# bridgedp/hunter_bipedal_control

Measured on NVIDIA H100. Metric: MPC+WBC control-step solves/sec (Hunter N=100), higher is better.
Workload: dtype f64

## Files before the change

hunter_bipedal_control_b200/csrc/hb_api.cu:

```cuda
#include <cuda_runtime.h>
#include <math.h>
#include <stdio.h>
#include <stdlib.h>
#include <string.h>

#include <new>

#include "../../include/hunter_b200.h"
#include "hb_common.cuh"
#include "hb_mpc.cuh"
#include "hb_planner.h"
#include <algorithm>
#include <climits>
#include <string>
#include <utility>
#include <atomic>
#include <mutex>
#include <cstring>
#include <thread>
#include <vector>
#include "hb_qp.cuh"
#include "hb_rbd.cuh"
#include "hb_sqp.cuh"
#include "hb_wbc.cuh"
// ... 214 lines not shown
      ctx_->base = (int)lo;
      rc = copy(lo, hi, true);
      if (!rc) rc = body(Chunk{c, lo, hi, (int)(hi - lo)});
      if (!rc) rc = copy(lo, hi, false);
    }
    ctx_->stream = ctx_->stream_main;
    ctx_->base = 0;
    return drain(ctx_, rc);
  }

 private:
  struct Slot { const void* src; void* dst; size_t bytes, count; void* dev; bool used; };
  template <class T> Dev<T> add(const void* src, void* dst, size_t per, size_t count, bool used) {
    Slot& s = s_[n_++];
    s = Slot{src, dst, per * sizeof(T), count, nullptr, used};
    return Dev<T>{&s.dev, per};
  }
  size_t place(void* base) {
    size_t off = 0;
    for (int k = 0; k < n_; ++k) if (s_[k].used) s_[k].dev = carve<char>(base, off, s_[k].bytes * s_[k].count);
    return off;
  }
  int copy(size_t lo, size_t hi, bool to_dev) {
    hb_ctx* ctx = ctx_;
    for (int k = 0; k < n_; ++k) {
      const Slot& s = s_[k];
      const size_t off = lo * s.bytes, n = (hi - lo) * s.bytes;
      if (to_dev && s.src) CK(cudaMemcpyAsync(static_cast<char*>(s.dev) + off, static_cast<const char*>(s.src) + off, n, cudaMemcpyHostToDevice, ctx->stream));
      if (!to_dev && s.dst) CK(cudaMemcpyAsync(static_cast<char*>(s.dst) + off, static_cast<char*>(s.dev) + off, n, cudaMemcpyDeviceToHost, ctx->stream));
    }
    return HB_OK;
  }
  hb_ctx* ctx_;
  size_t B_;
  Slot s_[16];
  int n_ = 0;
};

int cycle_chunks(const hb_ctx* ctx, int B, bool overlap) {
  const int c = ctx->cfg.e2e_chunks;
  return c > 0 ? (B >= 64 * c ? c : 1) : ((overlap && B >= 4096) ? 2 : 1);
}

}

extern "C" {

int hb_default_config(hb_config* cfg) {
  if (!cfg) return HB_EINVAL;
  cfg->horizon_N = 100;
  cfg->dt = 0.01;
  cfg->max_batch = 1024;
  cfg->wbc_rho = 1e-8;
  cfg->qp_max_iter = 40;
  cfg->line_search_max_trials = 14;
  cfg->time_horizon = 0.0;
  cfg->event_nodes = 0;
  cfg->e2e_chunks = 0;
  return HB_OK;
}

const char* hb_strerror(int code) {
  switch (code) {
    case HB_OK: return "ok";
    case HB_EINVAL: return "invalid argument";
    case HB_ECUDA: return "CUDA error";
    case HB_ENOMEM: return "out of memory";
    case HB_ECAP: return "batch exceeds context capacity";
    case HB_EPLAN: return "reference planner: swing phase without take-off / touch-down time, or reference capacity exceeded";
    case HB_ECOMM: return "NCCL not available or a collective failed (hb_shard_last_error)";
    default: return "unknown error";
  }
}

int hb_create(const hb_config* cfg, int device, hb_ctx** out) {
  if (!cfg || !out || cfg->horizon_N < 1 || cfg->horizon_N > HB_MAX_HORIZON || cfg->max_batch < 1 || !(cfg->dt > 0.0) || cfg->time_horizon < 0.0) return HB_EINVAL;
  hb_ctx* ctx = new (std::nothrow) hb_ctx();
  if (!ctx) return HB_ENOMEM;
  memset(ctx, 0, sizeof(*ctx));
  ctx->cfg = *cfg;
  ctx->device = device;
  hb_default_wbc_settings(&ctx->wbc);
  if (cudaSetDevice(device) != cudaSuccess) { hb_destroy(ctx); return HB_ECUDA; }
  if (cudaStreamCreateWithFlags(&ctx->stream, cudaStreamNonBlocking) != cudaSuccess) { ctx->stream = nullptr; hb_destroy(ctx); return HB_ECUDA; }
  ctx->stream_main = ctx->stream;
  if (cudaStreamCreateWithFlags(&ctx->stream_aux, cudaStreamNonBlocking) != cudaSuccess) { ctx->stream_aux = nullptr; hb_destroy(ctx); return HB_ECUDA; }
  Model* m = new Model();
  memset(m, 0, sizeof(Model));
  for (int b = 0; b < NBODY; ++b) {
    for (int i = 0; i < 3; ++i) { m->joint_xyz[3 * b + i] = HB_JOINT_XYZ[3 * b + i]; m->com[3 * b + i] = HB_BODY_COM[3 * b + i]; }
    for (int i = 0; i < 9; ++i) m->inertia[9 * b + i] = HB_BODY_INERTIA[9 * b + i];
    m->mass[b] = HB_BODY_MASS[b];
    int code = 0;
    for (int i = 0; i < 3; ++i) if (HB_JOINT_AXIS[3 * b + i] != 0.0) code = (HB_JOINT_AXIS[3 * b + i] > 0 ? 1 : -1) * (i + 1);
    m->joint_axis[b] = code;
  }
  m->total_mass = HB_TOTAL_MASS;
  for (int i = 0; i < 12; ++i) m->contact_offset[i] = HB_CONTACT_OFFSET[i];
  for (int j = 0; j < NJ; ++j) { m->joint_lower[j] = HB_JOINT_LOWER[j]; m->joint_upper[j] = HB_JOINT_UPPER[j]; m->joint_vel_limit[j] = HB_JOINT_VEL_LIMIT[j]; m->torque_limit[j] = HB_WBC_TORQUE_LIMITS[j % 5]; }
  for (int i = 0; i < NX; ++i) m->Q[i] = HB_Q_DIAG[i];
  cudaError_t e = cudaMemcpyToSymbol(c_model, m, sizeof(Model));
  if (e == cudaSuccess) {
    double* dR = nullptr;
    e = dalloc(&dR, NU * NU);
    if (e == cudaSuccess) {
      init_input_cost_kernel<<<1, 32, 0, ctx->stream>>>(dR);
      e = cudaStreamSynchronize(ctx->stream);
      if (e == cudaSuccess) e = cudaMemcpy(m->R, dR, sizeof(double) * NU * NU, cudaMemcpyDeviceToHost);
      if (e == cudaSuccess) e = cudaMemcpyToSymbol(c_model, m, sizeof(Model));
      cudaFree(dR);
    }
  }
  if (e == cudaSuccess) {
    double tab[32 * LQ_LANE_TAB] = {};
    for (int l = 0; l < 32; ++l) {
      double* t = tab + l * LQ_LANE_TAB;
      if (l < NX) t[0] = m->Q[l];
      if (l < 12) t[1] = m->R[l * NU + l];
      if (l >= 12 && l < NU) for (int j = 0; j < NJ; ++j) t[2 + j] = m->R[l * NU + 12 + j];
      if (l < 10) { t[12] = m->joint_lower[l]; t[13] = m->joint_upper[l]; }
      else if (l < 20) { t[12] = -m->joint_vel_limit[l - 10]; t[13] = m->joint_vel_limit[l - 10]; }
    }
    e = cudaMemcpyToSymbol(g_lq_lane, tab, sizeof(tab));
  }
  delete m;
  if (e != cudaSuccess) { ctx->last_cuda = (int)e; hb_destroy(ctx); return HB_ECUDA; }
  const size_t B = cfg->max_batch, N = cfg->horizon_N;
  const int rc = reserve_group(&ctx->scratch_mem, [&](void* m) {
    size_t off = 0;
    ctx->dxt = carve<double>(m, off, B * (N + 1) * NX); ctx->dut = carve<double>(m, off, B * N * NU);
    ctx->perf = carve<double>(m, off, B * 4); ctx->flags = carve<int32_t>(m, off, B);
    ctx->xdes = carve<double>(m, off, B * NX); ctx->udes = carve<double>(m, off, B * NU);
    ctx->wstatus = carve<int32_t>(m, off, B); ctx->witers = carve<int32_t>(m, off, B); ctx->wmode = carve<int32_t>(m, off, B);
    ctx->cyc_xref = carve<double>(m, off, B * (N + 1) * NX); ctx->cyc_swing = carve<double>(m, off, B * (N + 1) * 24);
    ctx->cyc_mode = carve<int32_t>(m, off, B * (N + 1)); ctx->cyc_tk = carve<double>(m, off, B * (N + 1)); ctx->cyc_nn = carve<int32_t>(m, off, B);
    ctx->res = carve_solution(m, off, B, N);
    ctx->res_sol = carve<double>(m, off, B * NWBC); ctx->res_stance = carve<double>(m, off, B * 12);
    return off;
  });
  if (rc) { hb_destroy(ctx); return rc; }
  {
    cudaError_t fe = cudaSuccess;
    auto attr = [&](const void* fn, size_t bytes) { if (fe == cudaSuccess) fe = cudaFuncSetAttribute(fn, cudaFuncAttributeMaxDynamicSharedMemorySize, (int)bytes); };
    attr((const void*)probe_flow_map_kernel, sizeof(ProbeShared));
    attr((const void*)qp_batch_kernel, 200 * 1024);
    attr((const void*)wbc_fused_kernel, wbc_fused_doubles() * sizeof(double));
    attr((const void*)hoqp_kernel, hoqp_smem_bytes());
    attr((const void*)hwbc_fused_kernel, hwbc_fused_bytes());
    attr((const void*)lin_kernel, 4 * sizeof(LinHalf) + sizeof(ChainModel));
    attr((const void*)lq_kernel, sizeof(LqShared));
    attr((const void*)riccati_kernel, sizeof(RicShared));
    attr((const void*)forward_linesearch2_kernel, sizeof(Fw2Shared));
    attr((const void*)warm_shift_kernel, sizeof(double) * ((HB_MAX_HORIZON + 1) * NX + HB_MAX_HORIZON * NU));
    for (const void* fn : {(const void*)wbc_fused_kernel, (const void*)riccati_kernel, (const void*)lq_kernel, (const void*)hwbc_fused_kernel})
      if (fe == cudaSuccess) fe = cudaFuncSetAttribute(fn, cudaFuncAttributePreferredSharedMemoryCarveout, (int)cudaSharedmemCarveoutMaxShared);
    if (fe != cudaSuccess) { ctx->last_cuda = (int)fe; hb_destroy(ctx); return HB_ECUDA; }
  }
  *out = ctx;
  return HB_OK;
}

int hb_destroy(hb_ctx* ctx) {
  if (!ctx) return HB_EINVAL;
  cudaSetDevice(ctx->device);
  void* const mem[] = {ctx->scratch_mem, ctx->sqp_mem, ctx->hoqp_mem, ctx->ro_mem, ctx->re_mem, ctx->goal_mem, ctx->pol_mem, ctx->odom_mem, ctx->arena,
                       ctx->pushes.dev, ctx->variations.dev, ctx->terrains.dev, ctx->goals.dev, ctx->plan_targets.dev, ctx->latencies.dev,
                       ctx->odometry.dev};
  for (void* p : mem) if (p) cudaFree(p);
  if (ctx->pinned) cudaFreeHost(ctx->pinned);
  if (ctx->prof_ev) { for (int i = 0; i < 2 * PROF_MAX; ++i) cudaEventDestroy(ctx->prof_ev[i]); delete[] ctx->prof_ev; delete[] ctx->prof_kind; }
  if (ctx->stream_aux) cudaStreamDestroy(ctx->stream_aux);
  if (ctx->stream_main) cudaStreamDestroy(ctx->stream_main);
  else if (ctx->stream) cudaStreamDestroy(ctx->stream);
  delete ctx;
  return HB_OK;
}

int hb_sync(hb_ctx* ctx) {
  if (!ctx) return HB_EINVAL;
  CK(cudaStreamSynchronize(ctx->stream));
  return HB_OK;
}
int hb_profile_enable(hb_ctx* ctx, int on) {
  if (!ctx) return HB_EINVAL;
  if (set_device(ctx)) return HB_ECUDA;
  if (on && !ctx->prof_ev) {
    ctx->prof_ev = new (std::nothrow) cudaEvent_t[2 * PROF_MAX];
    ctx->prof_kind = new (std::nothrow) int[PROF_MAX];
    if (!ctx->prof_ev || !ctx->prof_kind) return HB_ENOMEM;
    for (int i = 0; i < 2 * PROF_MAX; ++i) CK(cudaEventCreate(&ctx->prof_ev[i]));
  }
  ctx->prof_on = on ? 1 : 0;
  ctx->prof_n = 0;
  return HB_OK;
}

int hb_profile_read(hb_ctx* ctx, double* ms_per_kind, int64_t* count_per_kind) {
  if (!ctx || !ms_per_kind || !count_per_kind) return HB_EINVAL;
  if (set_device(ctx)) return HB_ECUDA;
  CK(cudaStreamSynchronize(ctx->stream));
  for (int k = 0; k < K_NKINDS; ++k) { ms_per_kind[k] = 0.0; count_per_kind[k] = 0; }
  for (int i = 0; i < ctx->prof_n; ++i) {
    float ms = 0.f;
    CK(cudaEventElapsedTime(&ms, ctx->prof_ev[2 * i], ctx->prof_ev[2 * i + 1]));
    ms_per_kind[ctx->prof_kind[i]] += ms;
    count_per_kind[ctx->prof_kind[i]]++;
  }
  ctx->prof_n = 0;
  return HB_OK;
}

const char* hb_last_cuda_error(const hb_ctx* ctx) { return ctx ? cudaGetErrorString((cudaError_t)ctx->last_cuda) : "no context"; }

int64_t hb_launch_count(const hb_ctx* ctx) { return ctx ? ctx->launches : 0; }
int64_t hb_last_reference_upload_bytes(const hb_ctx* ctx) { return ctx ? (int64_t)ctx->last_h2d_bytes : 0; }
void* hb_stream(hb_ctx* ctx) { return ctx ? (void*)ctx->stream : nullptr; }

static int launch_qp(hb_ctx* ctx, int B, int n, int m, const double* H, const double* g, const double* A, const double* lbA, const double* ubA,
                     size_t sH, size_t sA, size_t sB, const int32_t* m_per, double* x, int32_t* status, int32_t* iters) {
  if (!qp_shape_ok(n, m)) return HB_EINVAL;
  const size_t per_warp = qp_workspace_doubles(n) * sizeof(double);
  int wpb = (int)((200 * 1024) / per_warp);
  if (wpb < 1) return HB_EINVAL;
  if (wpb > 1) wpb = 1;
  const int blocks = (B + wpb - 1) / wpb;
  return launch(ctx, K_QP, qp_batch_kernel, blocks, 32 * wpb, per_warp * wpb, B, n, m, H, g, A, lbA, ubA, sH, sA, sB, m_per, ctx->cfg.wbc_rho,
                ctx->cfg.qp_max_iter, x, status, iters);
}

int hb_wbc_qp_batch_dev(hb_ctx* ctx, int B, int n, int m, const double* H, const double* g, const double* A, const double* lbA,
                        const double* ubA, double* x, int32_t* status, int32_t* iters) {
  ENTER(ctx, B, H && g && A && lbA && ubA && x, UNCAPPED);
  return launch_qp(ctx, B, n, m, H, g, A, lbA, ubA, (size_t)n * n, (size_t)m * n, (size_t)m, nullptr, x, status, iters);
}

int hb_wbc_solve_batch_dev(hb_ctx* ctx, int B, const double* x_des, const double* u_des, const double* rbd, const int32_t* mode,
                           const uint8_t* stance_mode, double* sol, int32_t* status) {
  ENTER(ctx, B, x_des && u_des && rbd && mode && sol, CAPPED);
  return launch(ctx, K_QP, wbc_fused_kernel, B, 32, wbc_fused_doubles() * sizeof(double), B, ctx->wbc, x_des, u_des, rbd, mode, stance_mode,
                ctx->cfg.wbc_rho, ctx->cfg.qp_max_iter, sol, status ? status : ctx->wstatus + ctx->base, ctx->witers + ctx->base);
}

int hb_wbc_assemble_batch_dev(hb_ctx* ctx, int B, const double* x_des, const double* u_des, const double* rbd, const int32_t* mode,
                              const uint8_t* stance_mode, double* H, double* g, double* A, double* lbA, double* ubA, int32_t* m_rows) {
  ENTER(ctx, B, x_des && u_des && rbd && mode && H && g && A && lbA && ubA && m_rows, UNCAPPED);
  const int wpb = 4;
  return launch(ctx, K_WBC_ASSEMBLE, wbc_assemble_kernel, (B + wpb - 1) / wpb, 32 * wpb, sizeof(WbcShared) * wpb, B, ctx->wbc, x_des, u_des, rbd, mode,
                stance_mode, H, g, A, lbA, ubA, m_rows);
}

int hb_wbc_qp_rows_batch_dev(hb_ctx* ctx, int B, int n, int m_alloc, const int32_t* m_rows, const double* H, const double* g, const double* A,
                             const double* lbA, const double* ubA, double* x, int32_t* status, int32_t* iters) {
  ENTER(ctx, B, m_rows && H && g && A && lbA && ubA && x, UNCAPPED);
  return launch_qp(ctx, B, n, m_alloc, H, g, A, lbA, ubA, (size_t)n * n, (size_t)m_alloc * n, (size_t)m_alloc, m_rows, x, status, iters);
}

static int hoqp_reserve(hb_ctx* ctx) {
  const size_t Bc = ctx->cfg.max_batch;
  return reserve_group(&ctx->hoqp_mem, [&](void* m) {
    size_t off = 0;
    ctx->hoqp_scratch = carve<double>(m, off, Bc * HQ_SCRATCH);
    return off;
  });
}

int hb_hoqp_solve_batch_dev(hb_ctx* ctx, int B, const hb_hoqp_problem* problems, double* x, double* slack, int32_t* status) {
  ENTER(ctx, B, problems && x, CAPPED);
  const int rc = hoqp_reserve(ctx);
  if (rc) return rc;
  return launch(ctx, K_QP, hoqp_kernel, B, 32, hoqp_smem_bytes(), B, problems, ctx->hoqp_scratch, 2 * ctx->cfg.qp_max_iter, x, slack, status);
}

static int hwbc_tasks_dev(hb_ctx* ctx, int B, const double* x_des, const double* u_des, const double* rbd, const int32_t* mode, hb_hoqp_problem* problems) {
  return launch(ctx, K_WBC_ASSEMBLE, hwbc_tasks_kernel, B, 32, 0, B, ctx->wbc, x_des, u_des, rbd, mode, problems);
}

int hb_hierarchical_wbc_solve_batch_dev(hb_ctx* ctx, int B, const double* x_des, const double* u_des, const double* rbd, const int32_t* mode, double* sol,
                                        int32_t* status) {
  ENTER(ctx, B, x_des && u_des && rbd && mode && sol, CAPPED);
  return launch(ctx, K_QP, hwbc_fused_kernel, B, 32, hwbc_fused_bytes(), B, ctx->wbc, x_des, u_des, rbd, mode, 2 * ctx->cfg.qp_max_iter, sol, status);
}

static int controller_wbc_dev(hb_ctx* ctx, int B, const double* x_des, const double* u_des, const double* rbd, const int32_t* mode,
                              const uint8_t* stance_mode, double* sol, int32_t* status) {
  if (ctx->wbc_form == HB_WBC_HIERARCHICAL)
    return hb_hierarchical_wbc_solve_batch_dev(ctx, B, x_des, u_des, rbd, mode, sol, status ? status : ctx->wstatus + ctx->base);
  return hb_wbc_solve_batch_dev(ctx, B, x_des, u_des, rbd, mode, stance_mode, sol, status);
}

int hb_mpc_cold_start_batch_dev(hb_ctx* ctx, int B, const double* x0, const int32_t* mode, double* x_traj, double* u_traj) {
  ENTER(ctx, B, x0 && mode && x_traj && u_traj, UNCAPPED);
  return launch(ctx, K_UNPROFILED, cold_start_kernel, B, 128, 0, B, ctx->cfg.horizon_N, x0, mode, x_traj, u_traj);
}

static int mpc_solve_impl(hb_ctx* ctx, int B, const double* x0, const double* x_ref, const double* swing_ref, const int32_t* mode,
                          double* x_traj, double* u_traj, hb_solve_info* info, const double* tk, const int32_t* nn) {
  ENTER(ctx, B, x0 && x_ref && swing_ref && mode && x_traj && u_traj && (tk == nullptr) == (nn == nullptr), CAPPED);
  const size_t Bc = ctx->cfg.max_batch, Nc = ctx->cfg.horizon_N;
  int rc = reserve_group(&ctx->sqp_mem, [&](void* m) {
    size_t off = 0;
    ctx->lin = carve<double>(m, off, Bc * Nc * LIN_STRIDE); ctx->proj = carve<double>(m, off, Bc * Nc * PJ_STRIDE);
    ctx->rk = carve<double>(m, off, Bc * Nc * RK_STRIDE);
    return off;
  });
  if (rc) return rc;
  SqpArgs a;
  a.tk = tk; a.nn = nn;
// ... 1209 lines not shown
```

hunter_bipedal_control_b200/csrc/hb_mpc.cuh:

```cuda
#pragma once
#include "hb_common.cuh"
#include "hb_rbd.cuh"

namespace hb {

constexpr int TS = NX * NX;
constexpr int NDIR = 13;

struct Pen { double v, d1, d2; };
__device__ __forceinline__ Pen relaxed_barrier(double h, double mu, double delta) {
  Pen p;
  if (h > delta) { p.v = -mu * log(h); p.d1 = -mu / h; p.d2 = mu / (h * h); }
  else {
    const double z = (h - 2.0 * delta) / delta;
    p.v = mu * (-log(delta) + 0.5 * z * z - 0.5);
    p.d1 = mu * (h - 2.0 * delta) / (delta * delta);
    p.d2 = mu / (delta * delta);
  }
  return p;
}
__device__ __forceinline__ Pen double_sided(double h, double lo, double hi, double mu, double delta) {
  const Pen a = relaxed_barrier(h - lo, mu, delta), b = relaxed_barrier(hi - h, mu, delta);
  Pen p; p.v = a.v + b.v; p.d1 = a.d1 - b.d1; p.d2 = a.d2 + b.d2;
  return p;
}

__device__ inline void flow_map_lane(const double* x, const double* u, double* f, double* epos, double* evel) {
  const Model& md = c_model;
  const double m = md.total_mass;
  double R0[9], ax0[9];
  {
    double sz, cz, sy, cy, sx, cx;
    sincos_t(x[9], sz, cz); sincos_t(x[10], sy, cy); sincos_t(x[11], sx, cx);
    R0[0] = cz * cy; R0[1] = cz * sy * sx - sz * cx; R0[2] = cz * sy * cx + sz * sx;
    R0[3] = sz * cy; R0[4] = sz * sy * sx + cz * cx; R0[5] = sz * sy * cx - cz * sx;
    R0[6] = -sy;     R0[7] = cy * sx;                R0[8] = cy * cx;
    ax0[0] = 0.0; ax0[1] = 0.0; ax0[2] = 1.0;
    ax0[3] = -sz; ax0[4] = cz; ax0[5] = 0.0;
    ax0[6] = cz * cy; ax0[7] = sz * cy; ax0[8] = -sy;
  }
  const double p0[3] = {x[6], x[7], x[8]};
  double P[3] = {0, 0, 0}, Lo[3] = {0, 0, 0}, mc[3] = {0, 0, 0};
  double IO[6] = {0, 0, 0, 0, 0, 0};
  double cp[12], cvj[12];
  auto add_inertia = [&](int b, const double* R, const double* cw) {
    const double mb = md.mass[b];
    const double* I = &md.inertia[9 * b];
    double T[9];
#pragma unroll
    for (int i = 0; i < 3; ++i)
#pragma unroll
      for (int k = 0; k < 3; ++k) T[3 * i + k] = R[3 * i] * I[k] + R[3 * i + 1] * I[3 + k] + R[3 * i + 2] * I[6 + k];
    const double c2 = cw[0] * cw[0] + cw[1] * cw[1] + cw[2] * cw[2];
    IO[0] += T[0] * R[0] + T[1] * R[1] + T[2] * R[2] + mb * (c2 - cw[0] * cw[0]);
    IO[1] += T[0] * R[3] + T[1] * R[4] + T[2] * R[5] - mb * cw[0] * cw[1];
    IO[2] += T[0] * R[6] + T[1] * R[7] + T[2] * R[8] - mb * cw[0] * cw[2];
    IO[3] += T[3] * R[3] + T[4] * R[4] + T[5] * R[5] + mb * (c2 - cw[1] * cw[1]);
    IO[4] += T[3] * R[6] + T[4] * R[7] + T[5] * R[8] - mb * cw[1] * cw[2];
    IO[5] += T[6] * R[6] + T[7] * R[7] + T[8] * R[8] + mb * (c2 - cw[2] * cw[2]);
#pragma unroll
    for (int i = 0; i < 3; ++i) mc[i] += cw[i] * mb;
  };
  {
    double r[3], cw[3];
    rot_const(R0, &md.com[0], r);
#pragma unroll
    for (int i = 0; i < 3; ++i) cw[i] = p0[i] + r[i];
    add_inertia(0, R0, cw);
  }
  for (int leg = 0; leg < 2; ++leg) {
    double R[9], p[3], w[3] = {0, 0, 0}, vl[3] = {0, 0, 0};
#pragma unroll
    for (int i = 0; i < 9; ++i) R[i] = R0[i];
#pragma unroll
    for (int i = 0; i < 3; ++i) p[i] = p0[i];
    for (int j = 0; j < 5; ++j) {
      const int b = 1 + 5 * leg + j;
      double d[3], wxd[3], a[3], sj, cj;
      rot_const(R, &md.joint_xyz[3 * b], d);
      cross(w, d, wxd);
#pragma unroll
      for (int i = 0; i < 3; ++i) { p[i] += d[i]; vl[i] += wxd[i]; }
      sincos_t(x[11 + b], sj, cj);
      joint_rotate_sc(R, md.joint_axis[b], sj, cj, a);
      const double vb = u[11 + b];
#pragma unroll
      for (int i = 0; i < 3; ++i) w[i] += a[i] * vb;
      double r[3], wxr[3], vc[3], cw[3], l[3], wl[3], Iwl[3], Iw[3];
      rot_const(R, &md.com[3 * b], r);
      cross(w, r, wxr);
      const double mb = md.mass[b];
#pragma unroll
      for (int i = 0; i < 3; ++i) { vc[i] = (vl[i] + wxr[i]) * mb; cw[i] = p[i] + r[i]; }
      cross(cw, vc, l);
      rotT(R, w, wl);
      const double* I = &md.inertia[9 * b];
#pragma unroll
      for (int i = 0; i < 3; ++i) Iwl[i] = wl[0] * I[3 * i] + wl[1] * I[3 * i + 1] + wl[2] * I[3 * i + 2];
      rot(R, Iwl, Iw);
#pragma unroll
      for (int i = 0; i < 3; ++i) { P[i] += vc[i]; Lo[i] += l[i] + Iw[i]; }
      add_inertia(b, R, cw);
    }
#pragma unroll
    for (int t = 0; t < 2; ++t) {
      const int c = leg + 2 * t;
      double off[3], wxo[3];
      rot_const(R, &md.contact_offset[3 * c], off);
      cross(w, off, wxo);
#pragma unroll
      for (int i = 0; i < 3; ++i) { cp[3 * c + i] = p[i] + off[i]; cvj[3 * c + i] = vl[i] + wxo[i]; }
    }
  }
  const double im = 1.0 / m;
  double com[3], cxP[3], hj[6];
#pragma unroll
  for (int i = 0; i < 3; ++i) com[i] = mc[i] * im;
  cross(com, P, cxP);
#pragma unroll
  for (int i = 0; i < 3; ++i) { hj[i] = P[i]; hj[3 + i] = Lo[i] - cxP[i]; }
  const double cc = com[0] * com[0] + com[1] * com[1] + com[2] * com[2];
  const double Ic[9] = {IO[0] - m * (cc - com[0] * com[0]), IO[1] + m * com[0] * com[1], IO[2] + m * com[0] * com[2],
                        IO[1] + m * com[0] * com[1], IO[3] - m * (cc - com[1] * com[1]), IO[4] + m * com[1] * com[2],
                        IO[2] + m * com[0] * com[2], IO[4] + m * com[1] * com[2], IO[5] - m * (cc - com[2] * com[2])};
  const double rb[3] = {com[0] - p0[0], com[1] - p0[1], com[2] - p0[2]};
  double Ae[6][3];
#pragma unroll
  for (int c = 0; c < 3; ++c) {
    const double* wc = &ax0[3 * c];
    double wxr[3];
    cross(wc, rb, wxr);
#pragma unroll
    for (int i = 0; i < 3; ++i) { Ae[i][c] = m * wxr[i]; Ae[3 + i][c] = Ic[3 * i] * wc[0] + Ic[3 * i + 1] * wc[1] + Ic[3 * i + 2] * wc[2]; }
  }
  double rl[3], ra[3];
  for (int i = 0; i < 3; ++i) { rl[i] = m * x[i] - hj[i]; ra[i] = m * x[3 + i] - hj[3 + i]; }
  const double a = Ae[3][0], b = Ae[3][1], c = Ae[3][2], d = Ae[4][0], e = Ae[4][1], g = Ae[4][2], h = Ae[5][0], k = Ae[5][1], l = Ae[5][2];
  const double det = a * (e * l - g * k) - b * (d * l - g * h) + c * (d * k - e * h);
  const double id = 1.0 / det;
  double th[3];
  th[0] = ((e * l - g * k) * ra[0] - (b * l - c * k) * ra[1] + (b * g - c * e) * ra[2]) * id;
  th[1] = (-(d * l - g * h) * ra[0] + (a * l - c * h) * ra[1] - (a * g - c * d) * ra[2]) * id;
  th[2] = ((d * k - e * h) * ra[0] - (a * k - b * h) * ra[1] + (a * e - b * d) * ra[2]) * id;
  double vb[6];
  for (int i = 0; i < 3; ++i) { vb[i] = (rl[i] - Ae[i][0] * th[0] - Ae[i][1] * th[1] - Ae[i][2] * th[2]) / m; vb[3 + i] = th[i]; }
  if (evel) {
    double W[3];
#pragma unroll
    for (int i = 0; i < 3; ++i) W[i] = ax0[i] * th[0] + ax0[3 + i] * th[1] + ax0[6 + i] * th[2];
#pragma unroll
    for (int cc2 = 0; cc2 < NC; ++cc2) {
      const double rr[3] = {cp[3 * cc2] - p0[0], cp[3 * cc2 + 1] - p0[1], cp[3 * cc2 + 2] - p0[2]};
      double wxr[3];
      cross(W, rr, wxr);
#pragma unroll
      for (int i = 0; i < 3; ++i) evel[3 * cc2 + i] = cvj[3 * cc2 + i] + vb[i] + wxr[i];
    }
  }
  if (epos) for (int i = 0; i < 12; ++i) epos[i] = cp[i];
  double fl[3] = {0, 0, 0}, fa[3] = {0, 0, 0};
  for (int cc2 = 0; cc2 < NC; ++cc2) {
    const double* F = u + 3 * cc2;
    const double r0 = cp[3 * cc2] - com[0], r1 = cp[3 * cc2 + 1] - com[1], r2 = cp[3 * cc2 + 2] - com[2];
    fl[0] += F[0]; fl[1] += F[1]; fl[2] += F[2];
    fa[0] += r1 * F[2] - r2 * F[1]; fa[1] += r2 * F[0] - r0 * F[2]; fa[2] += r0 * F[1] - r1 * F[0];
  }
  for (int i = 0; i < 3; ++i) { f[i] = fl[i] * im; f[3 + i] = fa[i] * im; }
  f[2] -= HB_GRAVITY;
  for (int i = 0; i < 6; ++i) f[6 + i] = vb[i];
  for (int j = 0; j < NJ; ++j) f[12 + j] = u[12 + j];
}

struct BarrierSum {
  double prod = 1.0, quad = 0.0;
  __device__ __forceinline__ void add(double h, double delta) {
    if (h > delta) prod *= h;
    else { const double z = (h - 2.0 * delta) / delta; quad += -log(delta) + 0.5 * z * z - 0.5; }
  }
  __device__ __forceinline__ double value(double mu) const { return mu * (quad - log(prod)); }
};

__device__ inline void node_values_lane(const double* x, const double* u, const double* xref, const double* swing, int mode,
                                        const double* epos, const double* evel, double& cost, double& eq_sq) {
  const Model& md = c_model;
  bool fl[4]; int ns = 0;
  for (int c = 0; c < 4; ++c) { fl[c] = contact_flag(mode, c); ns += fl[c]; }
  double cst = 0.0;
  for (int i = 0; i < NX; ++i) { const double d = x[i] - xref[i]; cst += 0.5 * md.Q[i] * d * d; }
  double du[NU];
  const double fz = ns > 0 ? md.total_mass * HB_GRAVITY / ns : 0.0;
  for (int i = 0; i < NU; ++i) du[i] = u[i];
  for (int c = 0; c < 4; ++c) if (fl[c]) du[3 * c + 2] -= fz;
  for (int i = 0; i < NU; ++i) { double s = 0.0; for (int j = 0; j < NU; ++j) s += md.R[i * NU + j] * du[j]; cst += 0.5 * du[i] * s; }
  double e2 = 0.0;
  BarrierSum fric, lpos, lvel, lforce;
  for (int c = 0; c < 4; ++c) {
    if (fl[c]) {
      const double Fx = u[3 * c], Fy = u[3 * c + 1], Fz = u[3 * c + 2];
      const double h = HB_FRICTION_MU * Fz - sqrt(Fx * Fx + Fy * Fy + HB_FRICTION_REGULARIZATION);
      fric.add(h, HB_FRICTION_BARRIER_DELTA);
      const double e0 = evel[3 * c], e1 = evel[3 * c + 1], e2z = evel[3 * c + 2] + HB_ZEROVEL_Z_GAIN * epos[3 * c + 2] + HB_ZEROVEL_Z_OFFSET;
      e2 += e0 * e0 + e1 * e1 + e2z * e2z;
    } else {
      for (int a = 0; a < 2; ++a) {
        const double h = evel[3 * c + a] - swing[6 * c + 3 + a] + HB_XY_POSITION_GAIN * (epos[3 * c + a] - swing[6 * c + a]);
        cst += 0.5 * HB_SOFT_SWING_WEIGHT * h * h;
      }
      const double en = evel[3 * c + 2] - swing[6 * c + 5] + HB_POSITION_ERROR_GAIN * (epos[3 * c + 2] - swing[6 * c + 2]);
      e2 += u[3 * c] * u[3 * c] + u[3 * c + 1] * u[3 * c + 1] + u[3 * c + 2] * u[3 * c + 2] + en * en;
    }
  }
  for (int j = 0; j < NJ; ++j) {
    lpos.add(x[12 + j] - md.joint_lower[j], HB_LIMIT_POS_DELTA); lpos.add(md.joint_upper[j] - x[12 + j], HB_LIMIT_POS_DELTA);
    lvel.add(u[12 + j] + md.joint_vel_limit[j], HB_LIMIT_VEL_DELTA); lvel.add(md.joint_vel_limit[j] - u[12 + j], HB_LIMIT_VEL_DELTA);
  }
  for (int c = 0; c < 4; ++c) { lforce.add(u[3 * c + 2], HB_LIMIT_FORCE_DELTA); lforce.add(HB_LIMIT_FORCE_MAX - u[3 * c + 2], HB_LIMIT_FORCE_DELTA); }
  cst += fric.value(HB_FRICTION_BARRIER_MU) + lpos.value(HB_LIMIT_POS_MU) + lvel.value(HB_LIMIT_VEL_MU) + lforce.value(HB_LIMIT_FORCE_MU);
  cost = cst; eq_sq = e2;
}


}

namespace {
using namespace hb;
__global__ void init_input_cost_kernel(double* Rout) {
  __shared__ double J0[12 * 16];
  const int lane = threadIdx.x;
  if (lane < 16) {
    double q[NQ], e[NQ];
    const double q0[NQ] = {HB_INITIAL_STATE[6], HB_INITIAL_STATE[7], HB_INITIAL_STATE[8], HB_INITIAL_STATE[9], HB_INITIAL_STATE[10], HB_INITIAL_STATE[11],
                           HB_INITIAL_STATE[12], HB_INITIAL_STATE[13], HB_INITIAL_STATE[14], HB_INITIAL_STATE[15], HB_INITIAL_STATE[16], HB_INITIAL_STATE[17],
                           HB_INITIAL_STATE[18], HB_INITIAL_STATE[19], HB_INITIAL_STATE[20], HB_INITIAL_STATE[21]};
    for (int i = 0; i < NQ; ++i) { q[i] = q0[i]; e[i] = (i == lane) ? 1.0 : 0.0; }
    KinOut<double> o;
    kin_pass<double>(q, e, o);
    for (int r = 0; r < 12; ++r) J0[r * 16 + lane] = o.cvel[r];
  }
  __syncthreads();
  const double rts[24] = {HB_R_TASKSPACE_DIAG[0], HB_R_TASKSPACE_DIAG[1], HB_R_TASKSPACE_DIAG[2], HB_R_TASKSPACE_DIAG[3], HB_R_TASKSPACE_DIAG[4], HB_R_TASKSPACE_DIAG[5],
                          HB_R_TASKSPACE_DIAG[6], HB_R_TASKSPACE_DIAG[7], HB_R_TASKSPACE_DIAG[8], HB_R_TASKSPACE_DIAG[9], HB_R_TASKSPACE_DIAG[10], HB_R_TASKSPACE_DIAG[11],
                          HB_R_TASKSPACE_DIAG[12], HB_R_TASKSPACE_DIAG[13], HB_R_TASKSPACE_DIAG[14], HB_R_TASKSPACE_DIAG[15], HB_R_TASKSPACE_DIAG[16], HB_R_TASKSPACE_DIAG[17],
                          HB_R_TASKSPACE_DIAG[18], HB_R_TASKSPACE_DIAG[19], HB_R_TASKSPACE_DIAG[20], HB_R_TASKSPACE_DIAG[21], HB_R_TASKSPACE_DIAG[22], HB_R_TASKSPACE_DIAG[23]};
  for (int idx = lane; idx < NU * NU; idx += 32) {
    const int i = idx / NU, j = idx - i * NU;
    double v = 0.0;
    if (i < 12 && i == j) v = rts[i];
    if (i >= 12 && j >= 12) for (int r = 0; r < 12; ++r) v += J0[r * 16 + 6 + i - 12] * rts[12 + r] * J0[r * 16 + 6 + j - 12];
    Rout[idx] = v;
  }
}
}
```

hunter_bipedal_control_b200/csrc/hb_sqp.cuh:

```cuda
#pragma once
#include "hb_common.cuh"
#include "hb_mpc.cuh"
#include "hb_rbd.cuh"

namespace hb {

constexpr int LIN_F1 = 0, LIN_F2 = 22, LIN_A1 = 44, LIN_A2 = 242, LIN_BF1 = 440, LIN_BF2 = 476, LIN_BV1 = 512, LIN_BV2 = 572,
              LIN_EPOS = 632, LIN_EVEL = 644, LIN_DPQ = 656, LIN_DVX = 812, LIN_DVV = 1076, LIN_STRIDE = 1200;
constexpr int NTMAX = 16;
constexpr int NVMAX = 8;
constexpr int PJ_BT = 0, PJ_AT = 144, PJ_PXV = 342, PJ_NV = 562, PJ_BTV = 642, PJ_QV = 664, PJ_RV = 686, PJ_META = 702, PJ_PEV = 710,
              PJ_QT = 720, PJ_PT = 1204, PJ_RF = 1380, PJ_RN = 1416, PJ_STRIDE = 1480;
constexpr int PJ_RT_PACKED = PJ_STRIDE - PJ_RF;
static_assert(PJ_AT + 9 * NX == PJ_PXV && PJ_RN + NVMAX * NVMAX == PJ_STRIDE && PJ_PEV + NJ == PJ_QT, "projected record blocks are contiguous");
static_assert(PJ_QT % 2 == 0 && PJ_PT % 2 == 0 && PJ_RF % 2 == 0 && PJ_STRIDE % 2 == 0, "bulk-copied blocks start on 16 bytes");
constexpr int RK_STRIDE = NTMAX * NX + NTMAX;

struct LinHalf {
  double x[NX], u[NU], x2[NX], f[NX];
  double Acm[6 * 16], Jc[12 * 16], dp[12 * NDIR], dv[12 * NDIR];
  double Abinv[36], AbinvAj[6 * NJ], vgen[16], epos[12], evel[12], com[3];
  double sn[NDIR], cs[NDIR];
  double dh[6 * NDIR], dcom[3 * NDIR], dvb[6 * NDIR];
  double vals[2 * 6];
// ... 1030 lines not shown
      const double* rp = sh.Huu + HUU_RP;
#pragma unroll
      for (int j = 0; j < NTP; ++j) {
        if (g.force(i) && g.force(j) && i / 3 == j / 3) c[j] = rp[9 * (i / 3) + (i % 3) * 3 + j % 3];
        else if (g.null(i) && g.null(j)) c[j] = rp[PJ_RN - PJ_RF + (i - g.nf) * NVMAX + j - g.nf];
        else if (i == j && !g.data(i)) c[j] = 1.0;
      }
      __syncwarp((1u << NTP) - 1u);
      if (g.force(i)) acc_rows(c, [&](int) { return g.dtim; }, SB + (i % 3) * SB_LD, SB_LD, 1);
      if (g.data(i)) acc_rows(c, [&](int k) { return in.Bt9[k * NTMAX + i]; }, SB + 3 * SB_LD, SB_LD, 9);
      if (g.null(i)) acc_rows(c, [&](int k) { return g.dt * in.Nv[k * NVMAX + i - g.nf]; }, SB + 12 * SB_LD, SB_LD, NJ);
    });
    if (lane < NTP) {
      double s0 = g.data(lane) ? in.rt[lane] : 0.0;
      if (g.force(lane)) s0 = fma(g.dtim, sh.sb[lane % 3], s0);
      if (g.data(lane)) {
#pragma unroll
        for (int k = 0; k < 9; ++k) s0 = fma(in.Bt9[k * NTMAX + lane], sh.sb[3 + k], s0);
      }
      if (g.null(lane)) {
#pragma unroll
        for (int k = 0; k < NJ; ++k) s0 = fma(g.dt * in.Nv[k * NVMAX + lane - g.nf], sh.sb[12 + k], s0);
      }
      sh.hu[lane] = s0;
    }
  }
  __syncthreads();
  if (warp == 0) {
    {
      double a[NTP], rinv = 0.0;
#pragma unroll
      for (int c = 0; c < NTP; ++c) a[c] = (lane < NTP && c <= lane) ? 0.5 * (sh.Huu[lane * 18 + c] + sh.Huu[c * 18 + lane]) : 0.0;
#pragma unroll
      for (int j = 0; j < NTP; ++j) {
        double d = __shfl_sync(HB_FULL_MASK, a[j], j);
        if (!(d > 0.0)) { fail = true; d = 1.0; }
        const double r = rsqrt(d);
        if (lane == j) rinv = r;
        const double l = a[j] * r;
        a[j] = l;
#pragma unroll
        for (int k = j + 1; k < NTP; ++k) a[k] = fma(-l, __shfl_sync(HB_FULL_MASK, l, k), a[k]);
      }
      double col[NTP], y[NTP];
#pragma unroll
      for (int c = 0; c < NTP; ++c) {
        double sacc = (lane < NX) ? sh.Hux[c * NX + lane] : ((lane == NX) ? sh.hu[c] : 0.0);
#pragma unroll
        for (int kk = 0; kk < c; ++kk) sacc = fma(-__shfl_sync(HB_FULL_MASK, a[kk], c), y[kk], sacc);
        y[c] = sacc * __shfl_sync(HB_FULL_MASK, rinv, c);
      }
#pragma unroll
      for (int c = NTP - 1; c >= 0; --c) {
        double sacc = y[c];
#pragma unroll
        for (int kk = c + 1; kk < NTP; ++kk) sacc = fma(-__shfl_sync(HB_FULL_MASK, a[c], kk), col[kk], sacc);
        col[c] = sacc * __shfl_sync(HB_FULL_MASK, rinv, c);
      }
      if (lane < NX) {
#pragma unroll
        for (int c = 0; c < NTP; ++c) { K[c * NX + lane] = -col[c]; rk[c * NX + lane] = -col[c]; }
      } else if (lane == NX) {
#pragma unroll
        for (int c = 0; c < NTP; ++c) { sh.kff[c] = -col[c]; rk[NTMAX * NX + c] = -col[c]; }
      }
    }
    __syncwarp();
    if (lane < NX) {
      double s0 = in.qt[lane], s1 = 0.0;
      if (lane == 1) s1 = s1 + sh.sb[1];
      else if (lane < 3) s0 = s0 + sh.sb[lane];
#pragma unroll
      for (int k = 3; k < NX; ++k) {
        if (k & 1) s1 = fma(in.At3[(k - 3) * NX + lane], sh.sb[k], s1);
        else s0 = fma(in.At3[(k - 3) * NX + lane], sh.sb[k], s0);
      }
#pragma unroll
      for (int c = 0; c < NTP; ++c) s0 = fma(sh.Hux[c * NX + lane], sh.kff[c], s0);
      sh.sv[lane] = s0 + s1;
    }
  } else {
    mbar_wait(&sh.bar[3], ph);
    __syncwarp();
    tri_tile<3, 4>(lane, [&](int i, int j) { return 0.5 * (sh.S[i * NX + j] + sh.S[j * NX + i]); },
                   [&](double (&c)[3][4], int i0, int j0, int mi, int nj) {
#pragma unroll
      for (int r = 0; r < 3; ++r) {
#pragma unroll
        for (int j = 0; j < 4; ++j) if (i0 + r < 3 && j < nj) c[r][j] = c[r][j] + sh.SA[(i0 + r) * NX + j0 + j];
      }
      acc_tile(c, in.At3 + i0, NX, mi, sh.SA + 3 * NX + j0, NX, nj, 19);
    }, [&](int i, int j, double v) { sh.S[i * NX + j] = v; });
  }
  __syncthreads();
  tri_tile<3, 2>((int)threadIdx.x, [&](int i, int j) { return sh.S[i * NX + j]; },
                 [&](double (&c)[3][2], int i0, int j0, int mi, int nj) { acc_tile(c, sh.Hux + i0, NX, mi, K + j0, NX, nj, NTP); },
                 [&](int i, int j, double v) { sh.S[i * NX + j] = v; if (j < i) sh.S[j * NX + i] = v; });
  __syncthreads();
}

__global__ void __launch_bounds__(64, 8) riccati_kernel(SqpArgs a) {
  extern __shared__ __align__(16) unsigned char smem_raw[];
  RicShared& sh = *reinterpret_cast<RicShared*>(smem_raw);
  const int inst = blockIdx.x, lane = threadIdx.x & 31, warp = threadIdx.x >> 5;
  const double* proj = a.proj + (size_t)inst * a.N * PJ_STRIDE;
  const int N = sqp_nn(a, inst);
  if (threadIdx.x == 0) { for (int b = 0; b < 4; ++b) mbar_init(&sh.bar[b], 1); }
  __syncthreads();
  if (warp == 1 && lane == 0) ric_prefetch_tma(sh.in[(N - 1) & 1], proj + (size_t)(N - 1) * PJ_STRIDE, &sh.bar[(N - 1) & 1]);
  unsigned ph_in0 = 0u, ph_in1 = 0u;
  for (int idx = threadIdx.x; idx < TS; idx += 64) sh.S[idx] = 0.0;
  if (threadIdx.x < NX) sh.sv[threadIdx.x] = 0.0;
  bool fail = false;
  double merit = 0.0, dyn = 0.0, eqs = 0.0;
  __syncthreads();
  for (int k = N - 1; k >= 0; --k) {
    const double* rec = proj + (size_t)k * PJ_STRIDE;
    double* rk = a.rk + ((size_t)inst * a.N + k) * RK_STRIDE;
    const unsigned ph = (unsigned)(N - 1 - k) & 1u;
    if (k & 1) { mbar_wait(&sh.bar[1], ph_in1); ph_in1 ^= 1u; } else { mbar_wait(&sh.bar[0], ph_in0); ph_in0 ^= 1u; }
    RicNodeIn& in = sh.in[k & 1];
    const int nt = (int)in.meta[0], nf = (int)in.meta[1], nv = (int)in.meta[2];
    if (warp == 0) {
      if (lane == 0) {
        fence_proxy_async();
        mbar_expect_tx(&sh.bar[2], (unsigned)((nv * NX + PJ_RT_PACKED) * sizeof(double)));
        if (nv > 0) bulk_g2s(sh.Hux + nf * NX, rec + PJ_PT, nv * NX * sizeof(double), &sh.bar[2]);
        bulk_g2s(sh.Huu + HUU_RP, rec + PJ_RF, PJ_RT_PACKED * sizeof(double), &sh.bar[2]);
      }
    } else if (k > 0 && lane == 0) {
      ric_prefetch_tma(sh.in[(k - 1) & 1], proj + (size_t)(k - 1) * PJ_STRIDE, &sh.bar[(k - 1) & 1]);
    }
    merit += in.meta[3]; dyn += in.meta[4]; eqs += in.meta[5];
    if (in.meta[6] != 0.0) fail = true;
    if (nf == 12 && nt == nt_regular(12)) riccati_node<12, 12>(sh, in, rec, rk, fail, warp, ph);
    else if (nf == 6 && nt == nt_regular(6)) riccati_node<10, 6>(sh, in, rec, rk, fail, warp, ph);
    else if (nf == 0 && nt == nt_regular(0)) riccati_node<6, 0>(sh, in, rec, rk, fail, warp, ph);
    else riccati_node<NTMAX, -1>(sh, in, rec, rk, fail, warp, ph);
  }
  if (threadIdx.x == 0) {
    double* pf = a.perf + (size_t)inst * 4;
    pf[0] = merit; pf[1] = dyn; pf[2] = eqs; pf[3] = 0.0;
    a.flags[inst] = fail ? 1 : 0;
  }
}

struct FwNode {
  double Bt9[9 * NTMAX], At9[9 * NX], Pxv[NJ * NX], Nv[NJ * NVMAX], bt[NX], qt[NX], rt[NTMAX], meta[8], pev[NJ];
  double K[NTMAX * NX], kff[NTMAX], u[NU];
};
static_assert(offsetof(FwNode, At9) == PJ_AT * sizeof(double) && offsetof(FwNode, pev) == PJ_PEV * sizeof(double) &&
              offsetof(FwNode, K) == PJ_QT * sizeof(double) && offsetof(FwNode, u) == offsetof(FwNode, K) + RK_STRIDE * sizeof(double),
              "FwNode mirrors the record and the gains");
struct Fw2Shared {
  FwNode nd[2];
  double dx[NX], dxn[NX], w[NTMAX];
  unsigned long long bar[2];
};
static_assert(sizeof(FwNode) % 16 == 0 && (NJ * sizeof(double)) % 16 == 0 && (NJ * NX * sizeof(double)) % 16 == 0, "bulk copies need 16-byte multiples");

__device__ __forceinline__ void fw_prefetch_tma(FwNode& n, const double* __restrict__ rec, const double* __restrict__ rk, const double* __restrict__ uk,
                                                unsigned long long* bar) {
  fence_proxy_async();
  mbar_expect_tx(bar, (unsigned)sizeof(FwNode));
  bulk_g2s(n.Bt9, rec, PJ_QT * sizeof(double), bar);
  bulk_g2s(n.K, rk, RK_STRIDE * sizeof(double), bar);
  bulk_g2s(n.u, uk, sizeof(n.u), bar);
}

__global__ void __launch_bounds__(32) forward_linesearch2_kernel(SqpArgs a, int max_trials, void* info_out) {
  extern __shared__ __align__(16) unsigned char smem_raw[];
  Fw2Shared& sh = *reinterpret_cast<Fw2Shared*>(smem_raw);
  const int inst = blockIdx.x, lane = threadIdx.x, NS = a.N;
  const int N = sqp_nn(a, inst);
  double* xt = a.xt + (size_t)inst * (NS + 1) * NX;
  double* ut = a.ut + (size_t)inst * NS * NU;
  double* dxt = a.dxt + (size_t)inst * (NS + 1) * NX;
  double* dut = a.dut + (size_t)inst * NS * NU;
  const double* xref = a.x_ref + (size_t)inst * (NS + 1) * NX;
  const double* swing = a.swing + (size_t)inst * (NS + 1) * 24;
  const int32_t* mode = a.mode + (size_t)inst * (NS + 1);
  const double* proj = a.proj + (size_t)inst * NS * PJ_STRIDE;
  const double* rkb = a.rk + (size_t)inst * NS * RK_STRIDE;
  if (lane == 0) { mbar_init(&sh.bar[0], 1); mbar_init(&sh.bar[1], 1); }
  __syncwarp();
  if (lane == 0) fw_prefetch_tma(sh.nd[0], proj, rkb, ut, &sh.bar[0]);
  unsigned fph0 = 0u, fph1 = 0u;
  if (lane < NX) { xt[lane] = a.x0[(size_t)inst * NX + lane]; sh.dx[lane] = 0.0; dxt[lane] = 0.0; }
  double armijo = 0.0;
  bool finite = (a.flags[inst] == 0);
  const double im_mass = 1.0 / c_model.total_mass;
  for (int k = 0; k < N; ++k) {
    if (k + 1 < N && lane == 0) fw_prefetch_tma(sh.nd[(k + 1) & 1], proj + (size_t)(k + 1) * PJ_STRIDE, rkb + (size_t)(k + 1) * RK_STRIDE, ut + (k + 1) * NU, &sh.bar[(k + 1) & 1]);
    if (k & 1) { mbar_wait(&sh.bar[1], fph1); fph1 ^= 1u; } else { mbar_wait(&sh.bar[0], fph0); fph0 ^= 1u; }
    const FwNode& nd = sh.nd[k & 1];
    const int nt = (int)nd.meta[0], nf = (int)nd.meta[1], nv = (int)nd.meta[2];
    const int md_k = mode[k];
    const double dtk = sqp_dt(a, inst, k);
    unsigned fmask = 0u;
#pragma unroll
    for (int c = 0; c < 4; ++c) if (contact_flag(md_k, c)) fmask |= 7u << (3 * c);
    double arm = 0.0;
    if (lane < nt) {
      double s = nd.kff[lane];
#pragma unroll
      for (int j = 0; j < NX; ++j) s = fma(nd.K[lane * NX + j], sh.dx[j], s);
      sh.w[lane] = s;
      arm = nd.rt[lane] * s;
    }
    __syncwarp();
    if (lane < NX) {
      double du;
      if (lane < 12) {
        if (contact_flag(md_k, lane / 3)) du = sh.w[__popc(fmask & ((1u << lane) - 1u))];
        else du = -nd.u[lane];
      } else {
        const int i = lane - 12;
        du = nd.pev[i];
#pragma unroll
        for (int j = 0; j < NX; ++j) du = fma(nd.Pxv[i * NX + j], sh.dx[j], du);
        for (int c = 0; c < nv; ++c) du = fma(nd.Nv[i * NVMAX + c], sh.w[nf + c], du);
      }
      double s = nd.bt[lane];
      if (lane >= 3 && lane < 12) {
        const double* ar = nd.At9 + (lane - 3) * NX;
        const double* br = nd.Bt9 + (lane - 3) * NTMAX;
        double s1 = 0.0;
#pragma unroll
        for (int j = 0; j < NX; j += 2) { s = fma(ar[j], sh.dx[j], s); s1 = fma(ar[j + 1], sh.dx[j + 1], s1); }
        s += s1;
        for (int c = 0; c < nt; ++c) s = fma(br[c], sh.w[c], s);
      } else if (lane < 3) {
        double fsum = 0.0;
#pragma unroll
        for (int c = 0; c < 4; ++c) if (contact_flag(md_k, c)) fsum += sh.w[__popc(fmask & ((1u << (3 * c + lane)) - 1u))];
        s += sh.dx[lane] + (dtk * im_mass) * fsum;
      } else {
        s += sh.dx[lane] + dtk * (du - nd.pev[lane - 12]);
      }
      sh.dxn[lane] = s;
      dxt[(k + 1) * NX + lane] = s;
      arm += nd.qt[lane] * sh.dx[lane];
      dut[k * NU + lane] = du;
      if (!isfinite(s) || !isfinite(du)) finite = false;
    }
    armijo += warp_sum(arm);
    __syncwarp();
    if (lane < NX) sh.dx[lane] = sh.dxn[lane];
    __syncwarp();
  }
  finite = __all_sync(HB_FULL_MASK, finite);
  const double* pf = a.perf + (size_t)inst * 4;
  const double merit0 = pf[0], v0 = sqrt(pf[1] + pf[2]);
  const double gamma_c = 1e-6, armijoFactor = 1e-4, alpha_decay = 0.5, alpha_min = 1e-4;
  double alpha = 1.0, merit1 = merit0, v1 = v0;
  bool accepted = false;
  int trials = 0;
  if (finite) {
    while (alpha >= alpha_min && trials < max_trials) {
      double ms = 0.0, ds = 0.0, es = 0.0;
      for (int k = lane; k < N; k += 32) {
        const double dt = sqp_dt(a, inst, k);
        double x[NX], u[NU], xn[NX], f1[NX], f2[NX], x2[NX], ep[12], ev[12], xr[NX], sw[24];
        for (int i = 0; i < NX; ++i) { x[i] = xt[k * NX + i] + alpha * dxt[k * NX + i]; xn[i] = xt[(k + 1) * NX + i] + alpha * dxt[(k + 1) * NX + i]; xr[i] = xref[k * NX + i]; }
        for (int i = 0; i < NU; ++i) u[i] = ut[k * NU + i] + alpha * dut[k * NU + i];
        for (int i = 0; i < 24; ++i) sw[i] = swing[k * 24 + i];
        flow_map_lane(x, u, f1, ep, ev);
        for (int i = 0; i < NX; ++i) x2[i] = x[i] + dt * f1[i];
        flow_map_lane(x2, u, f2, nullptr, nullptr);
        double d2 = 0.0;
        for (int i = 0; i < NX; ++i) { const double d = x[i] + 0.5 * dt * (f1[i] + f2[i]) - xn[i]; d2 += d * d; }
        double cost, e2;
        node_values_lane(x, u, xr, sw, mode[k], ep, ev, cost, e2);
        ms += dt * cost; ds += dt * d2; es += dt * e2;
      }
      ms = warp_sum(ms); ds = warp_sum(ds); es = warp_sum(es);
      ++trials;
      const double vn = sqrt(ds + es);
      const double am = alpha * armijo;
      bool acc;
      if (vn > HB_SQP_G_MAX) acc = vn < (1.0 - gamma_c) * v0;
      else if (vn < HB_SQP_G_MIN && v0 < HB_SQP_G_MIN && am < 0.0) acc = ms < merit0 + armijoFactor * am;
      else acc = ms < (merit0 - gamma_c * v0) || vn < (1.0 - gamma_c) * v0;
      if (isfinite(ms) && isfinite(vn) && acc) { accepted = true; merit1 = ms; v1 = vn; break; }
      alpha *= alpha_decay;
    }
  }
  if (accepted) {
    auto axpy = [&](double* y, const double* d, int n) {
      int idx = lane;
      for (; idx + 96 < n; idx += 128) {
        const double y0 = y[idx], y1 = y[idx + 32], y2 = y[idx + 64], y3 = y[idx + 96];
        const double d0 = d[idx], d1 = d[idx + 32], d2 = d[idx + 64], d3 = d[idx + 96];
        y[idx] = fma(alpha, d0, y0); y[idx + 32] = fma(alpha, d1, y1); y[idx + 64] = fma(alpha, d2, y2); y[idx + 96] = fma(alpha, d3, y3);
      }
      for (; idx < n; idx += 32) y[idx] = fma(alpha, d[idx], y[idx]);
    };
    axpy(xt, dxt, (N + 1) * NX);
    axpy(ut, dut, N * NU);
  }
  if (lane == 0 && info_out) {
    struct Info { double alpha, merit0, merit1, viol0, viol1, armijo; int32_t status, n_trials; };
    Info* io = reinterpret_cast<Info*>(info_out) + inst;
    io->alpha = accepted ? alpha : 0.0; io->merit0 = merit0; io->merit1 = merit1; io->viol0 = v0; io->viol1 = v1;
    io->armijo = armijo; io->status = finite ? 0 : 3; io->n_trials = trials;
  }
}

}
```

Before: 190,700.

## Stage line-search per-lane state in shared memory columns to cut register spills

The line-search loop in forward_linesearch2_kernel now keeps each lane's trial state (x, u, contact positions and velocities, first RK stage, base rotation) in a strided shared-memory column. It reuses the FwNode buffers through a union. flow_map_lane and node_values_lane are templated on accessor types, so they read and write this shared storage directly, and RK2 stage points are computed on the fly instead of being materialised. Asm barriers keep the compiler from caching these values in registers. The aim is to remove local-memory spills from large per-thread arrays, at the cost of extra shared-memory traffic and a max-shared carveout for this kernel.

```diff
diff --git a/hunter_bipedal_control_b200/csrc/hb_api.cu b/hunter_bipedal_control_b200/csrc/hb_api.cu
--- a/hunter_bipedal_control_b200/csrc/hb_api.cu
+++ b/hunter_bipedal_control_b200/csrc/hb_api.cu
@@ -390,7 +390,8 @@
     attr((const void*)riccati_kernel, sizeof(RicShared));
     attr((const void*)forward_linesearch2_kernel, sizeof(Fw2Shared));
     attr((const void*)warm_shift_kernel, sizeof(double) * ((HB_MAX_HORIZON + 1) * NX + HB_MAX_HORIZON * NU));
-    for (const void* fn : {(const void*)wbc_fused_kernel, (const void*)riccati_kernel, (const void*)lq_kernel, (const void*)hwbc_fused_kernel})
+    for (const void* fn : {(const void*)wbc_fused_kernel, (const void*)riccati_kernel, (const void*)lq_kernel, (const void*)hwbc_fused_kernel,
+                           (const void*)forward_linesearch2_kernel})
       if (fe == cudaSuccess) fe = cudaFuncSetAttribute(fn, cudaFuncAttributePreferredSharedMemoryCarveout, (int)cudaSharedmemCarveoutMaxShared);
     if (fe != cudaSuccess) { ctx->last_cuda = (int)fe; hb_destroy(ctx); return HB_ECUDA; }
   }
diff --git a/hunter_bipedal_control_b200/csrc/hb_mpc.cuh b/hunter_bipedal_control_b200/csrc/hb_mpc.cuh
--- a/hunter_bipedal_control_b200/csrc/hb_mpc.cuh
+++ b/hunter_bipedal_control_b200/csrc/hb_mpc.cuh
@@ -25,7 +25,8 @@
   return p;
 }
 
-__device__ inline void flow_map_lane(const double* x, const double* u, double* f, double* epos, double* evel) {
+template <bool VEL, class XV, class UV, class CV>
+__device__ inline void flow_map_lane(const XV& x, const UV& u, double* f, CV epos, CV evel, CV r0) {
   const Model& md = c_model;
   const double m = md.total_mass;
   double R0[9], ax0[9];
@@ -42,7 +43,6 @@
   const double p0[3] = {x[6], x[7], x[8]};
   double P[3] = {0, 0, 0}, Lo[3] = {0, 0, 0}, mc[3] = {0, 0, 0};
   double IO[6] = {0, 0, 0, 0, 0, 0};
-  double cp[12], cvj[12];
   auto add_inertia = [&](int b, const double* R, const double* cw) {
     const double mb = md.mass[b];
     const double* I = &md.inertia[9 * b];
@@ -67,11 +67,13 @@
 #pragma unroll
     for (int i = 0; i < 3; ++i) cw[i] = p0[i] + r[i];
     add_inertia(0, R0, cw);
+#pragma unroll
+    for (int i = 0; i < 9; ++i) r0[i] = R0[i];
   }
   for (int leg = 0; leg < 2; ++leg) {
     double R[9], p[3], w[3] = {0, 0, 0}, vl[3] = {0, 0, 0};
 #pragma unroll
-    for (int i = 0; i < 9; ++i) R[i] = R0[i];
+    for (int i = 0; i < 9; ++i) R[i] = r0[i];
 #pragma unroll
     for (int i = 0; i < 3; ++i) p[i] = p0[i];
     for (int j = 0; j < 5; ++j) {
@@ -109,7 +111,7 @@
       rot_const(R, &md.contact_offset[3 * c], off);
       cross(w, off, wxo);
 #pragma unroll
-      for (int i = 0; i < 3; ++i) { cp[3 * c + i] = p[i] + off[i]; cvj[3 * c + i] = vl[i] + wxo[i]; }
+      for (int i = 0; i < 3; ++i) { epos[3 * c + i] = p[i] + off[i]; if (VEL) evel[3 * c + i] = vl[i] + wxo[i]; }
     }
   }
   const double im = 1.0 / m;
@@ -144,30 +146,32 @@
   th[2] = ((d * k - e * h) * ra[0] - (a * k - b * h) * ra[1] + (a * e - b * d) * ra[2]) * id;
   double vb[6];
   for (int i = 0; i < 3; ++i) { vb[i] = (rl[i] - Ae[i][0] * th[0] - Ae[i][1] * th[1] - Ae[i][2] * th[2]) / m; vb[3 + i] = th[i]; }
-  if (evel) {
+  if (VEL) {
     double W[3];
 #pragma unroll
     for (int i = 0; i < 3; ++i) W[i] = ax0[i] * th[0] + ax0[3 + i] * th[1] + ax0[6 + i] * th[2];
 #pragma unroll
     for (int cc2 = 0; cc2 < NC; ++cc2) {
-      const double rr[3] = {cp[3 * cc2] - p0[0], cp[3 * cc2 + 1] - p0[1], cp[3 * cc2 + 2] - p0[2]};
+      const double rr[3] = {epos[3 * cc2] - p0[0], epos[3 * cc2 + 1] - p0[1], epos[3 * cc2 + 2] - p0[2]};
       double wxr[3];
       cross(W, rr, wxr);
 #pragma unroll
-      for (int i = 0; i < 3; ++i) evel[3 * cc2 + i] = cvj[3 * cc2 + i] + vb[i] + wxr[i];
-    }
-  }
-  if (epos) for (int i = 0; i < 12; ++i) epos[i] = cp[i];
+      for (int i = 0; i < 3; ++i) evel[3 * cc2 + i] = evel[3 * cc2 + i] + vb[i] + wxr[i];
+    }
+  }
   double fl[3] = {0, 0, 0}, fa[3] = {0, 0, 0};
   for (int cc2 = 0; cc2 < NC; ++cc2) {
-    const double* F = u + 3 * cc2;
-    const double r0 = cp[3 * cc2] - com[0], r1 = cp[3 * cc2 + 1] - com[1], r2 = cp[3 * cc2 + 2] - com[2];
+    const double F[3] = {u[3 * cc2], u[3 * cc2 + 1], u[3 * cc2 + 2]};
+    const double r0 = epos[3 * cc2] - com[0], r1 = epos[3 * cc2 + 1] - com[1], r2 = epos[3 * cc2 + 2] - com[2];
     fl[0] += F[0]; fl[1] += F[1]; fl[2] += F[2];
     fa[0] += r1 * F[2] - r2 * F[1]; fa[1] += r2 * F[0] - r0 * F[2]; fa[2] += r0 * F[1] - r1 * F[0];
   }
+#pragma unroll
   for (int i = 0; i < 3; ++i) { f[i] = fl[i] * im; f[3 + i] = fa[i] * im; }
   f[2] -= HB_GRAVITY;
+#pragma unroll
   for (int i = 0; i < 6; ++i) f[6 + i] = vb[i];
+#pragma unroll
   for (int j = 0; j < NJ; ++j) f[12 + j] = u[12 + j];
 }
 
@@ -180,18 +184,28 @@
   __device__ __forceinline__ double value(double mu) const { return mu * (quad - log(prod)); }
 };
 
-__device__ inline void node_values_lane(const double* x, const double* u, const double* xref, const double* swing, int mode,
-                                        const double* epos, const double* evel, double& cost, double& eq_sq) {
+template <class XV, class UV, class CV>
+__device__ inline void node_values_lane(const XV& x, const UV& u, const double* xref, const double* swing, int mode, CV epos, CV evel,
+                                        double& cost, double& eq_sq) {
   const Model& md = c_model;
   bool fl[4]; int ns = 0;
+#pragma unroll
   for (int c = 0; c < 4; ++c) { fl[c] = contact_flag(mode, c); ns += fl[c]; }
   double cst = 0.0;
   for (int i = 0; i < NX; ++i) { const double d = x[i] - xref[i]; cst += 0.5 * md.Q[i] * d * d; }
   double du[NU];
   const double fz = ns > 0 ? md.total_mass * HB_GRAVITY / ns : 0.0;
+#pragma unroll
   for (int i = 0; i < NU; ++i) du[i] = u[i];
+#pragma unroll
   for (int c = 0; c < 4; ++c) if (fl[c]) du[3 * c + 2] -= fz;
-  for (int i = 0; i < NU; ++i) { double s = 0.0; for (int j = 0; j < NU; ++j) s += md.R[i * NU + j] * du[j]; cst += 0.5 * du[i] * s; }
+#pragma unroll
+  for (int i = 0; i < NU; ++i) {
+    double s = 0.0;
+#pragma unroll
+    for (int j = 0; j < NU; ++j) s += md.R[i * NU + j] * du[j];
+    cst += 0.5 * du[i] * s;
+  }
   double e2 = 0.0;
   BarrierSum fric, lpos, lvel, lforce;
   for (int c = 0; c < 4; ++c) {
diff --git a/hunter_bipedal_control_b200/csrc/hb_sqp.cuh b/hunter_bipedal_control_b200/csrc/hb_sqp.cuh
--- a/hunter_bipedal_control_b200/csrc/hb_sqp.cuh
+++ b/hunter_bipedal_control_b200/csrc/hb_sqp.cuh
@@ -1206,12 +1206,36 @@
 static_assert(offsetof(FwNode, At9) == PJ_AT * sizeof(double) && offsetof(FwNode, pev) == PJ_PEV * sizeof(double) &&
               offsetof(FwNode, K) == PJ_QT * sizeof(double) && offsetof(FwNode, u) == offsetof(FwNode, K) + RK_STRIDE * sizeof(double),
               "FwNode mirrors the record and the gains");
+constexpr int LS_X = 0, LS_U = 22, LS_EP = 44, LS_EV = 56, LS_F1 = 68, LS_R0 = 80, LS_SLOTS = 89;
 struct Fw2Shared {
-  FwNode nd[2];
+  union {
+    FwNode nd[2];
+    double ls[LS_SLOTS * 32];
+  };
   double dx[NX], dxn[NX], w[NTMAX];
   unsigned long long bar[2];
 };
 static_assert(sizeof(FwNode) % 16 == 0 && (NJ * sizeof(double)) % 16 == 0 && (NJ * NX * sizeof(double)) % 16 == 0, "bulk copies need 16-byte multiples");
+static_assert(8 * (sizeof(Fw2Shared) + 1024) <= 228 * 1024, "forward_linesearch2_kernel: 8 blocks per SM (one wave of 1024 instances)");
+
+struct LsColumn {
+  double* ls; int off;
+  __device__ __forceinline__ double& operator[](int i) const { return ls[off + i * 32]; }
+  __device__ __forceinline__ LsColumn at(int slot) const { return LsColumn{ls, off + slot * 32}; }
+  __device__ __forceinline__ LsColumn fresh() const {
+    LsColumn c = *this;
+    asm volatile("" : "+r"(c.off));
+    return c;
+  }
+};
+struct Rk2Stage1 {
+  LsColumn col;
+  __device__ __forceinline__ double operator[](int i) const { return i < 12 ? col[LS_F1 + i] : col[LS_U + i]; }
+};
+struct Rk2Point {
+  LsColumn col; double dt;
+  __device__ __forceinline__ double operator[](int i) const { return col[LS_X + i] + dt * Rk2Stage1{col}[i]; }
+};
 
 __device__ __forceinline__ void fw_prefetch_tma(FwNode& n, const double* __restrict__ rec, const double* __restrict__ rk, const double* __restrict__ uk,
                                                 unsigned long long* bar) {
@@ -1311,21 +1335,45 @@
   bool accepted = false;
   int trials = 0;
   if (finite) {
+    const LsColumn col{sh.ls, lane};
     while (alpha >= alpha_min && trials < max_trials) {
       double ms = 0.0, ds = 0.0, es = 0.0;
       for (int k = lane; k < N; k += 32) {
         const double dt = sqp_dt(a, inst, k);
-        double x[NX], u[NU], xn[NX], f1[NX], f2[NX], x2[NX], ep[12], ev[12], xr[NX], sw[24];
-        for (int i = 0; i < NX; ++i) { x[i] = xt[k * NX + i] + alpha * dxt[k * NX + i]; xn[i] = xt[(k + 1) * NX + i] + alpha * dxt[(k + 1) * NX + i]; xr[i] = xref[k * NX + i]; }
-        for (int i = 0; i < NU; ++i) u[i] = ut[k * NU + i] + alpha * dut[k * NU + i];
-        for (int i = 0; i < 24; ++i) sw[i] = swing[k * 24 + i];
-        flow_map_lane(x, u, f1, ep, ev);
-        for (int i = 0; i < NX; ++i) x2[i] = x[i] + dt * f1[i];
-        flow_map_lane(x2, u, f2, nullptr, nullptr);
+        {
+          const LsColumn c0 = col.fresh();
+#pragma unroll
+          for (int i = 0; i < NX; ++i) c0[LS_X + i] = xt[k * NX + i] + alpha * dxt[k * NX + i];
+#pragma unroll
+          for (int i = 0; i < NU; ++i) c0[LS_U + i] = ut[k * NU + i] + alpha * dut[k * NU + i];
+        }
+        double f[NX];
+        {
+          const LsColumn c1 = col.fresh();
+          flow_map_lane<true>(c1.at(LS_X), c1.at(LS_U), f, c1.at(LS_EP), c1.at(LS_EV), c1.at(LS_R0));
+#pragma unroll
+          for (int i = 0; i < 12; ++i) c1[LS_F1 + i] = f[i];
+        }
+        double cost, e2;
+        {
+          const LsColumn c2 = col.fresh();
+          node_values_lane(c2.at(LS_X), c2.at(LS_U), xref + k * NX, swing + k * 24, mode[k], c2.at(LS_EP), c2.at(LS_EV), cost, e2);
+        }
+        {
+          const LsColumn c3 = col.fresh();
+          flow_map_lane<false>(Rk2Point{c3, dt}, c3.at(LS_U), f, c3.at(LS_EP), c3.at(LS_EV), c3.at(LS_R0));
+        }
         double d2 = 0.0;
-        for (int i = 0; i < NX; ++i) { const double d = x[i] + 0.5 * dt * (f1[i] + f2[i]) - xn[i]; d2 += d * d; }
-        double cost, e2;
-        node_values_lane(x, u, xr, sw, mode[k], ep, ev, cost, e2);
+        {
+          const LsColumn c4 = col.fresh();
+          const Rk2Stage1 f1{c4};
+#pragma unroll
+          for (int i = 0; i < NX; ++i) {
+            const double xn = xt[(k + 1) * NX + i] + alpha * dxt[(k + 1) * NX + i];
+            const double d = c4[LS_X + i] + 0.5 * dt * (f1[i] + f[i]) - xn;
+            d2 += d * d;
+          }
+        }
         ms += dt * cost; ds += dt * d2; es += dt * e2;
       }
       ms = warp_sum(ms); ds = warp_sum(ds); es = warp_sum(es);
```

Result: no change. 191,500, median of 6 (+0.4%).
